# RNG65536/CUDA-volpath

Measured on AMD Instinct MI355X. Metric: Msamples/sec (WxHxspp) + achieved HBM GB/s, Julia 256^3 @ 800x600, higher is better.
Workload: dtype f32; 1 GPU; julia256_800x600_global_majorant; image=800x600, estimator=global_majorant, bound_brick=1, rng=philox2x32-7, parallelism=pixel-tiles x1

## Files before the change

### cuda-volpath_amd/csrc/vp_context.cpp

```cpp
#include "vp_state.h"

namespace vph __attribute__((visibility("hidden")))
{
State                      g_default;
static thread_local State* t_current = nullptr;
State& cur() { return t_current ? *t_current : g_default; }

int fail(int code, const char* fmt, ...)
{
    char    buf[512];
    va_list ap;
    va_start(ap, fmt);
    vsnprintf(buf, sizeof buf, fmt, ap);
    va_end(ap);
    G.err = buf;
    return code;
}
[[noreturn]] void die(const char* what)
{
    fprintf(stderr, "volpath_hip: %s: %s\n", what, G.err.c_str());
    exit(EXIT_FAILURE);
}
int ensure_device()
{
// ... 54 lines not shown
    if (knob("VP_CELL_BRICKS", 0, 1, v)) G.cell_bricks = (int)v;
    if (knob("VP_NO_CRAWL_TABLE", 0, 1, v)) G.use_crawl_table = v == 0;
    if (knob("VP_NO_EMPTY_TABLE", 0, 1, v)) G.use_empty_table = v == 0;
    if (knob("VP_NO_SUN_CLIP", 0, 1, v)) G.use_sun_clip = v == 0;
    if (knob("VP_DENSE_PERCENT", 0, 101, v)) G.dense_fraction = (float)v / 100.0f;
    if (knob("VP_NO_OPACITY_LDS", 0, 1, v)) G.opacity_lds = v == 0;
    if (knob("VP_NO_OPACITY_CELLS", 0, 1, v)) G.use_opacity_cells = v == 0;
    if (knob("VP_NO_LIGHT_CONST", 0, 1, v)) G.use_light_const = v == 0;
    if (knob("VP_NO_CONST_ROWS", 0, 1, v)) G.use_const_rows = v == 0;
    if (knob("VP_NO_APPROACH", 0, 1, v)) G.use_approach = v == 0;
    if (knob("VP_NO_APPROACH_LOCAL", 0, 1, v)) G.use_approach_local = v == 0;
    if (knob("VP_NO_APPROACH_TABLE", 0, 1, v)) G.use_approach_table = v == 0;
    if (knob("VP_NO_RAY_TABLE", 0, 1, v)) G.use_ray_table = v == 0;
    if (knob("VP_APPROACH_FRAMES_LOG2", 0, 6, v)) G.approach_fshift_max = (unsigned)v;
    if (knob("VP_APPROACH_STEPS", 0, 1 << 30, v)) G.approach_steps = (unsigned)v;
    if (knob("VP_NO_LIGHT", 0, 1, v)) G.use_light = v == 0;
    if (knob("VP_NO_LIGHT_OVERLAP", 0, 1, v)) G.light_overlap = v == 0;
    if (knob("VP_NO_LIGHT_LOCAL", 0, 1, v)) G.use_light_local = v == 0;
    if (knob("VP_DEBUG_ONLY_CLASS", 0, 1, v)) G.debug_only_class = (int)v;
    if (knob("VP_GENERAL_BLOCKS_PER_CU", 1, 8, v)) G.general_blocks_per_cu = (unsigned)v;
    if (knob("VP_LIGHT_BLOCKS_PER_CU", 1, 8, v)) G.light_blocks_per_cu = (unsigned)v;
    if (knob("VP_THR_TABLE", 2, 1 << 20, v)) G.thr_entries = (unsigned)v;
    if (knob("VP_LOOKAHEAD", 0, 4096, v)) G.la_max = (int)v;
    if (knob("VP_LOOKAHEAD_OVERLAP_FROM", 1, 4096, v)) G.la_overlap_from = (int)v;
    if (knob("VP_LOOKAHEAD_RAMP_FROM", 2, 4096, v)) G.la_ramp_from = (int)v;
    if (knob("VP_LOOKAHEAD_FLOOR", 1, 4096, v)) G.la_floor = (int)v;
    if (knob("VP_LOOKAHEAD_DIV", 1, 16, v)) G.la_div = (int)v;
    if (knob("VP_LOOKAHEAD_NO_SPECULATION", 0, 1, v)) G.la_speculate = v == 0;
    if (knob("VP_NO_LA_CANCEL", 0, 1, v)) G.la_cancel = v == 0;
    if (knob("VP_NO_PIPELINE", 0, 1, v)) G.pipeline = v == 0;
// ... 727 lines not shown
    if (!dm || !df) return fail(VP_E_NOMEM, "vp_test_log_forms: no device memory");
    HIPCHK(hipMemsetAsync(dm, 0, 8, G.stream));
    HIPCHK(hipMemsetAsync(df, 0xff, 4, G.stream));
    if (G.arith == VP_ARITH_FAST) launch_test_log_forms_fast(which, lo_bits, hi_bits, dm, df, G.stream);
    else launch_test_log_forms(which, lo_bits, hi_bits, dm, df, G.stream);
    HIPCHK(hipStreamSynchronize(G.stream));
    unsigned long long m = 0;
    HIPCHK(hipMemcpy(&m, dm, 8, hipMemcpyDeviceToHost));
    HIPCHK(hipMemcpy(first_bad, df, 4, hipMemcpyDeviceToHost));
    *mismatches = m;
    return VP_OK;
}
int vp_test_approach_walk(int kind, int n, const float* params, const uint32_t* script, const uint32_t* words, uint32_t n_words, uint32_t* out_new,
                          uint32_t* out_ref)
{
    if (kind < 0 || kind > 1) return fail(VP_E_ARG, "vp_test_approach_walk: unknown walk %d (0 approach_k's, 1 the local walks' inner loop)", kind);
    if (n < 0) return fail(VP_E_ARG, "vp_test_approach_walk: negative count %d", n);
    if (!params || !script || !out_new || !out_ref || (n_words && !words)) return fail(VP_E_ARG, "vp_test_approach_walk: null argument");
    for (int i = 0; i < n; i++)
        if (script[4 * (size_t)i + 1] > n_words || script[4 * (size_t)i + 2] > n_words - script[4 * (size_t)i + 1])
            return fail(VP_E_ARG, "vp_test_approach_walk: the script of case %d (%u words from %u) leaves the %u words given", i, script[4 * (size_t)i + 2],
                        script[4 * (size_t)i + 1], n_words);
    int rc = ensure_device();
    if (rc) return rc;
    if (n == 0) return VP_OK;
    DevArrays D;
    const size_t c = (size_t)n;
    float*    dp = (float*)D.get(c * 16);
    unsigned *ds = (unsigned*)D.get(c * 16), *dw = (unsigned*)D.get((size_t)n_words * 4), *dn = (unsigned*)D.get(c * 20), *dr = (unsigned*)D.get(c * 20);
    if (!dp || !ds || !dw || !dn || !dr) return fail(VP_E_NOMEM, "vp_test_approach_walk: no device memory");
    HIPCHK(hipMemcpy(dp, params, c * 16, hipMemcpyHostToDevice));
    HIPCHK(hipMemcpy(ds, script, c * 16, hipMemcpyHostToDevice));
    if (n_words) HIPCHK(hipMemcpy(dw, words, (size_t)n_words * 4, hipMemcpyHostToDevice));
    if (G.arith == VP_ARITH_FAST) launch_test_approach_walk_fast(kind, n, dp, ds, dw, dn, dr, G.stream);
    else launch_test_approach_walk(kind, n, dp, ds, dw, dn, dr, G.stream);
    HIPCHK(hipStreamSynchronize(G.stream));
    HIPCHK(hipMemcpy(out_new, dn, c * 20, hipMemcpyDeviceToHost));
    HIPCHK(hipMemcpy(out_ref, dr, c * 20, hipMemcpyDeviceToHost));
    return VP_OK;
}
int vp_test_sun_start(int n, const float* origin_xyz, const float* sun_dir, const float* box, uint32_t* out_new, uint32_t* out_ref)
{
    if (n < 0) return fail(VP_E_ARG, "vp_test_sun_start: negative count %d", n);
    if (!origin_xyz || !sun_dir || !box || !out_new || !out_ref) return fail(VP_E_ARG, "vp_test_sun_start: null argument");
    int rc = ensure_device();
    if (rc) return rc;
    if (n == 0) return VP_OK;
    DevArrays D;
    const size_t c = (size_t)n;
    float*    dor = (float*)D.get(c * 12), *db = (float*)D.get(24);
// ... 169 lines not shown
```

### cuda-volpath_amd/csrc/vp_integrator.h

```cpp
enum : int
{
    ST_DONE    = 0,
    ST_SETUP   = 1,
    ST_TRACK   = 2,
    ST_SHADOW  = 3,
    EV_SCATTER = 4,
    EV_NEE     = 5,
    EV_BG      = 6,
    EV_WRITE   = 7,
    EV_MIS     = 8,
    EV_HG      = 9
};

#ifndef VP_PAD_STEP
#define VP_PAD_STEP 0
#endif
#ifndef VP_PAD_FETCH
#define VP_PAD_FETCH 0
#endif
#ifndef VP_PAD_EOF
#define VP_PAD_EOF 0
#endif
#ifndef VP_PAD_SETUP
#define VP_PAD_SETUP 0
// ... 1224 lines not shown

__device__ __forceinline__ bool approach_cancelled(const LaunchDev& L)
{
    if (!L.cancel) return false;
    unsigned w = 0;
    if ((threadIdx.x & 63u) == 0u) w = __hip_atomic_load(L.cancel, __ATOMIC_RELAXED, __HIP_MEMORY_SCOPE_AGENT);
    return (unsigned)__builtin_amdgcn_readfirstlane((int)w) >= L.batch_id;
}
#define VP_KEEP_BRANCH() asm volatile("")
#define VP_WALK_UNROLL 2
__device__ __forceinline__ float walk_limit(float t_box, float t_empty) { return t_box < t_empty ? t_box : t_empty; }
__device__ __forceinline__ bool walks_backwards(float inv_sigma) { return (f2u(inv_sigma) >> 31) != 0u; }

template <class RNG>
__device__ __forceinline__ unsigned approach_walk(float& dist, const float t_lim, const float inv_sigma, const unsigned cap, RNG& rng, unsigned& sa,
                                                  unsigned& sb)
{
    unsigned steps = 0;
    rng.save(sa, sb);
    if (!RNG::kShadowSubstream || walks_backwards(inv_sigma))
    {
        for (; steps < cap; steps++)
        {
            const float d2 = dist + -logf_(rng.next_a()) * inv_sigma;
            if (!(d2 < t_lim)) break;
            dist = d2;
            (void)rng.next_b();
            rng.save(sa, sb);
        }
        return steps;
    }
    const unsigned base = sa;
    float          a = dist, b = dist;
    unsigned       twos = 0;
    bool           odd  = false;
    for (unsigned i = 0; i < cap; i += 2u)
    {
        rng.set_pair(base + i);
        const float ua = rng.next_a();
        b              = a + -logf_pos_(ua) * inv_sigma;
        if (ua == 0.0f || !(b < t_lim)) break;
        VP_KEEP_BRANCH();
        odd = true;
        if (i + 1u == cap) break;
        rng.set_pair(base + i + 1u);
        const float ub = rng.next_a();
        a              = b + -logf_pos_(ub) * inv_sigma;
        if (ub == 0.0f || !(a < t_lim)) break;
        VP_KEEP_BRANCH();
        odd = false;
        twos++;
    }
// ... 56 lines not shown
    before.set_pair(base + steps);
    before.save(ta, tb);
    return stopped && d2 >= t_far;
}

template <class RNG>
__global__ __launch_bounds__(256) void approach_k(SceneDev S, LaunchDev L)
{
    if (approach_cancelled(L)) return;
    const unsigned sh   = L.approach_fshift;
    const unsigned slot = blockIdx.x * (256u >> sh) + (threadIdx.x >> sh), fl = (blockIdx.y << sh) + (threadIdx.x & ((1u << sh) - 1u));
    if (slot >= L.nslots || fl >= (unsigned)L.nframes) return;
    const ParamDev& P = L.P;
    const unsigned pix = L.pixels[slot], px = pix & 0xffffu, py = pix >> 16;
    if (px >= P.width || py >= P.height) return;
    f3 ro, rd;
    camera_ray(S, P.width, P.height, px, py, ro, rd);
    float    t_near, tf, dist = 0.0f;
    unsigned pairs = 0, sa = 0, sb = 0;
    RNG      rng;
    if (intersect_box(ro, rd, S, t_near, tf))
    {
        if (t_near < 0.0f) t_near = 0.0f;
        dist                      = t_near;
        const float t_end         = tf;
        const float t_empty       = L.crawl[2 * ((size_t)px + (size_t)py * P.width) + 1].x;
        const float s             = hyperion_s(0 - 5);
        const float cur_density   = (1.0f - s) * P.density + s * P.density * (1.0f - P.g);
        const float sigma_t_prime = max3(f3{P.sigma_t[0], P.sigma_t[1], P.sigma_t[2]}) * cur_density;
        const float inv_sigma     = rcp_(sigma_t_prime);
        rng.init(px, py, (unsigned)(L.frame0 + (int)fl), L.key0, L.key1);
        pairs = approach_walk(dist, walk_limit(t_end, t_empty), inv_sigma, L.approach_steps, rng, sa, sb);
    }
    L.stage[(size_t)fl * L.stage_stride + L.slot_base + slot] = make_float4(dist, u2f(sa), u2f(sb), u2f(pairs));
    if (L.counters && pairs) atomicAdd(&L.counters[1], (unsigned long long)pairs);
}

template <class RNG, bool QUANT>
__global__ __launch_bounds__(256) void approach_local_k(SceneDev S, LaunchDev L)
{
    if (approach_cancelled(L)) return;
    const unsigned sh   = L.approach_fshift;
    const unsigned slot = blockIdx.x * (256u >> sh) + (threadIdx.x >> sh), fl = (blockIdx.y << sh) + (threadIdx.x & ((1u << sh) - 1u));
    if (slot >= L.nslots || fl >= (unsigned)L.nframes) return;
    const ParamDev& P = L.P;
    const unsigned pix = L.pixels[slot], px = pix & 0xffffu, py = pix >> 16;
    if (px >= P.width || py >= P.height) return;
// ... 123 lines not shown
```

### cuda-volpath_amd/csrc/vp_kernels.h

```cpp
#pragma once
#include <hip/hip_runtime.h>

#include "vp_device.h"

#define VP_BLOCK 256
#ifndef VP_BLOCK_LDS
#define VP_BLOCK_LDS 512
#endif
#ifndef VP_MIN_WAVES
#define VP_MIN_WAVES 1
#endif
#define VP_LDS_BYTES_PER_CU (160 * 1024)
#define VP_LDS_BOUND_ENTRIES 32768
#ifndef VP_CHUNK
#define VP_CHUNK 128
#endif
#define VP_NQUEUES 8
#define VP_QUEUE_STRIDE 16
#ifndef VP_WAIT_LANES
#define VP_WAIT_LANES 28
#endif
#ifndef VP_WAIT_ITERS
#define VP_WAIT_ITERS 16
#endif
// ... 61 lines not shown
    const unsigned char* exit_oct;
    int      exit_start;
    unsigned exit_nbytes;
    unsigned exit_bytes;
    unsigned* cancel;
    unsigned  batch_id;
    unsigned      const_from;
    const float4* stage_const;
    const unsigned* bound_codes;
    unsigned        bound_pal[2];
    const float4* seg_table;
    unsigned sub_shift;
    unsigned layers;
    const float4* ray;
    float4* groups;
};

[[noreturn]] void kernel_not_built();
constexpr int CENSUS_RENDER = 0, CENSUS_LAYERS = 1, CENSUS_APPROACH = 2;
void census_record(int unit, int kind, unsigned index);
size_t census_size(int kind);
void census_read(int unit, int kind, unsigned* launches, unsigned char* built, size_t count, bool reset);
void census_built(int kind, unsigned char* built, size_t count);
void census_built_fast(int kind, unsigned char* built, size_t count);
void groups_census_record(unsigned index);
void groups_census_read(unsigned* launches, unsigned char* built, size_t count, bool reset);
void group_layers_census_record(unsigned index);
void group_layers_census_read(unsigned* launches, unsigned char* built, size_t count, bool reset);
void launch_render(const SceneDev& S, const LaunchDev& L, int est, int rng, bool quant, bool half, bool count, int lds_form, bool mis, int trk,
                   int blocks, hipStream_t st);
// ... 69 lines not shown
void launch_relight_composite(float4* dst, const float4* sun, const float4* sky, const float4* trans, float3 sun_gain, float3 sky_gain, const float4* plate,
                              float r, float g, float b, int size, float s, hipStream_t st);
void launch_gamma(float4* dst, const float4* src, int size, float s, float inv_gamma, hipStream_t st);
void launch_accumulate(float4* dst, const float4* src, size_t n, hipStream_t st);
void launch_test_hg(const float* g, const float* r0, const float* r1, const float* nrm, const float* cosq, float* dir, float* ev, int n, hipStream_t st);
void launch_test_box(const SceneDev& S, const float* o, const float* d, int* hit, float* tn, float* tf, int n, hipStream_t st);
void launch_test_env(const SceneDev& S, const float* d, float* out, int n, hipStream_t st);
void launch_test_camera_ray(const SceneDev& S, unsigned width, unsigned height, const unsigned* pixels, float* dir, int n, hipStream_t st);
void launch_test_camera_ray_fast(const SceneDev& S, unsigned width, unsigned height, const unsigned* pixels, float* dir, int n, hipStream_t st);
void launch_test_math(int which, const float* in, float* out, int n, hipStream_t st);
void launch_test_roots(int which, unsigned lo, unsigned hi, unsigned long long* mismatches, unsigned* first_bad, hipStream_t st);
void launch_test_hg_fast(const float* g, const float* r0, const float* r1, const float* nrm, const float* cosq, float* dir, float* ev, int n, hipStream_t st);
void launch_test_math_fast(int which, const float* in, float* out, int n, hipStream_t st);
void launch_test_log_forms(int which, unsigned lo, unsigned hi, unsigned long long* mismatches, unsigned* first_bad, hipStream_t st);
void launch_test_log_forms_fast(int which, unsigned lo, unsigned hi, unsigned long long* mismatches, unsigned* first_bad, hipStream_t st);
void launch_test_approach_walk(int kind, int n, const float* par, const unsigned* scr, const unsigned* words, unsigned* out_new, unsigned* out_ref, hipStream_t st);
void launch_test_approach_walk_fast(int kind, int n, const float* par, const unsigned* scr, const unsigned* words, unsigned* out_new, unsigned* out_ref,
                                    hipStream_t st);
void launch_test_sun_start(int n, const float* origin, const float* sun_dir, const float* box, unsigned* out_new, unsigned* out_ref, hipStream_t st);
void launch_test_sun_start_fast(int n, const float* origin, const float* sun_dir, const float* box, unsigned* out_new, unsigned* out_ref, hipStream_t st);
void launch_test_rng(int mode, unsigned x, unsigned y, unsigned f, unsigned k0, unsigned k1, int n, float* out, hipStream_t st);
void launch_test_density(const SceneDev& S, bool quant, bool half, const float* pos, float* out, int n, hipStream_t st);
}
```

### cuda-volpath_amd/csrc/vp_kernels.hip

```cpp
#include <hip/hip_runtime.h>

#include <atomic>
#include <cmath>
#include <cstdint>
#include <cstdio>
#include <cstdlib>
#include <type_traits>
#include <utility>

#include "vp_device.h"
#include "vp_kernels.h"

namespace vp
{
#include "vp_integrator.h"

__global__ void thr_table_k(ParamDev P, float* table, unsigned count)
{
    if (threadIdx.x || blockIdx.x) return;
    const float max_sig       = max3(f3{P.sigma_t[0], P.sigma_t[1], P.sigma_t[2]});
    const float s             = hyperion_s(0 - 5);
    const float cur_density   = (1.0f - s) * P.density + s * P.density * (1.0f - P.g);
    const float sigma_t_prime = max_sig * cur_density;
    const float inv_sigma_t   = 1.0f / sigma_t_prime;
// ... 1671 lines not shown
{
    hipLaunchKernelGGL(test_env_k, dim3((n + 255) / 256), dim3(256), 0, st, S, d, out, n);
}
void launch_test_math(int which, const float* in, float* out, int n, hipStream_t st)
{
    hipLaunchKernelGGL(test_math_k, dim3((n + 255) / 256), dim3(256), 0, st, which, in, out, n);
}
void launch_test_roots(int which, unsigned lo, unsigned hi, unsigned long long* mismatches, unsigned* first_bad, hipStream_t st)
{
    hipLaunchKernelGGL(test_roots_k, dim3(2048), dim3(256), 0, st, which, lo, hi, mismatches, first_bad);
}
void launch_test_log_forms(int which, unsigned lo, unsigned hi, unsigned long long* mismatches, unsigned* first_bad, hipStream_t st)
{
    hipLaunchKernelGGL(test_log_forms_k, dim3(2048), dim3(256), 0, st, which, lo, hi, mismatches, first_bad);
}
void launch_test_approach_walk(int kind, int n, const float* par, const unsigned* scr, const unsigned* words, unsigned* out_new, unsigned* out_ref, hipStream_t st)
{
    hipLaunchKernelGGL(test_approach_walk_k, dim3((n + 63) / 64), dim3(64), 0, st, kind, n, par, scr, words, out_new, out_ref);
}
void launch_test_sun_start(int n, const float* origin, const float* sun_dir, const float* box, unsigned* out_new, unsigned* out_ref, hipStream_t st)
{
    hipLaunchKernelGGL(test_sun_start_k, dim3((n + 255) / 256), dim3(256), 0, st, n, origin, sun_dir[0], sun_dir[1], sun_dir[2], box, out_new, out_ref);
}
void launch_test_camera_ray(const SceneDev& S, unsigned width, unsigned height, const unsigned* pixels, float* dir, int n, hipStream_t st)
{
    hipLaunchKernelGGL(test_camera_ray_k, dim3((n + 255) / 256), dim3(256), 0, st, S, width, height, pixels, dir, n);
}
void launch_test_rng(int mode, unsigned x, unsigned y, unsigned f, unsigned k0, unsigned k1, int n, float* out, hipStream_t st)
{
    if (mode == RNG_PHILOX) hipLaunchKernelGGL(test_rng_k<RngPhilox>, dim3(1), dim3(64), 0, st, x, y, f, k0, k1, n, out);
    else if (mode == RNG_PHILOX7) hipLaunchKernelGGL(test_rng_k<RngPhilox7>, dim3(1), dim3(64), 0, st, x, y, f, k0, k1, n, out);
    else hipLaunchKernelGGL(test_rng_k<RngSamplerH>, dim3(1), dim3(64), 0, st, x, y, f, k0, k1, n, out);
}
// ... 8 lines not shown
```

### cuda-volpath_amd/csrc/vp_kernels_fast.hip

```cpp
#define VP_ARITH_FAST 1

#include <hip/hip_runtime.h>

#include <cstdio>
#include <cstdlib>
#include <utility>

#include "vp_device.h"
#include "vp_kernels.h"

namespace vp
{
namespace fast
{
#include "vp_integrator.h"
#include "vp_test_kernels.h"

#include "vp_dispatch.h"
}

void launch_render_fast(const SceneDev& S, const LaunchDev& L, int est, int rng, bool quant, bool half, bool count, int lds_form, bool mis, int trk,
                        int blocks, hipStream_t st)
{
    fast::dispatch_render(S, L, est, rng, quant, half, count, lds_form, mis, trk, blocks, st);
// ... 8 lines not shown
void census_built_fast(int kind, unsigned char* built, size_t count) { fast::dispatch_census_built(kind, built, count); }

void launch_test_hg_fast(const float* g, const float* r0, const float* r1, const float* nrm, const float* cosq, float* dir, float* ev, int n, hipStream_t st)
{
    hipLaunchKernelGGL(fast::test_hg_k, dim3((n + 255) / 256), dim3(256), 0, st, g, r0, r1, nrm, cosq, dir, ev, n);
}
void launch_test_math_fast(int which, const float* in, float* out, int n, hipStream_t st)
{
    hipLaunchKernelGGL(fast::test_math_k, dim3((n + 255) / 256), dim3(256), 0, st, which, in, out, n);
}
void launch_test_log_forms_fast(int which, unsigned lo, unsigned hi, unsigned long long* mismatches, unsigned* first_bad, hipStream_t st)
{
    hipLaunchKernelGGL(fast::test_log_forms_k, dim3(2048), dim3(256), 0, st, which, lo, hi, mismatches, first_bad);
}
void launch_test_approach_walk_fast(int kind, int n, const float* par, const unsigned* scr, const unsigned* words, unsigned* out_new, unsigned* out_ref,
                                    hipStream_t st)
{
    hipLaunchKernelGGL(fast::test_approach_walk_k, dim3((n + 63) / 64), dim3(64), 0, st, kind, n, par, scr, words, out_new, out_ref);
}
void launch_test_camera_ray_fast(const SceneDev& S, unsigned width, unsigned height, const unsigned* pixels, float* dir, int n, hipStream_t st)
{
    hipLaunchKernelGGL(fast::test_camera_ray_k, dim3((n + 255) / 256), dim3(256), 0, st, S, width, height, pixels, dir, n);
}
void launch_test_sun_start_fast(int n, const float* origin, const float* sun_dir, const float* box, unsigned* out_new, unsigned* out_ref, hipStream_t st)
{
    hipLaunchKernelGGL(fast::test_sun_start_k, dim3((n + 255) / 256), dim3(256), 0, st, n, origin, sun_dir[0], sun_dir[1], sun_dir[2], box, out_new, out_ref);
}
}
```

### cuda-volpath_amd/csrc/vp_render.cpp

```cpp
#include "vp_state.h"

namespace vph __attribute__((visibility("hidden")))
{
static float span_ms(hipEvent_t a, hipEvent_t b, hipEvent_t& end)
{
    float ms = 0.0f, since = 0.0f;
    if (hipEventElapsedTime(&ms, a, b) != hipSuccess) { (void)hipGetLastError(); return 0.0f; }
    if (end && hipEventElapsedTime(&since, end, b) == hipSuccess)
    {
        if (since <= 0.0f) return 0.0f;
        ms = std::min(ms, since);
    }
    else (void)hipGetLastError();
    end = b;
    return std::max(ms, 0.0f);
}
static void fold_span(hipEvent_t a, hipEvent_t b, hipEvent_t& end, double& sum)
{
    hipEvent_t e = end;
    if (hipEventQuery(b) == hipSuccess) sum += span_ms(a, b, e);
    else (void)hipGetLastError();
    put_event(a);
    if (e == b) { put_event(end); end = b; }
    else put_event(b);
// ... 312 lines not shown
}
static hipError_t launch_general_class(Launch& X, const ClassGrid& g)
{
    const LaunchPlan& A = X.A; LaunchDev& L = X.L; const Target& T = A.T;
    hipError_t le = hipSuccess;
    ClassTimer ct(0, T.stream);
    L.approach = 0;
    G.last_approach = 0;
    G.last_approach_table = 0;
    const bool aux_ok = !A.appr_aux_needed || T.rt->handover.p != nullptr;
    if (A.appr_aux_needed) L.approach_aux = T.rt->handover;
    if (A.approach && aux_ok && L.stage && X.f <= 65535)
    {
        L.approach       = A.approach_thr ? 2u : 1u;
        L.approach_steps = G.approach_steps;
        L.approach_fshift = 0;
        while (L.approach_fshift < G.approach_fshift_max && (2u << L.approach_fshift) <= (unsigned)X.f) L.approach_fshift++;
        X.k.approach(X.S, L, G.est, G.rng, G.quant, T.stream);
        le = hipGetLastError();
        G.last_approach = (int)L.approach;
        G.last_approach_table = (G.est == VP_EST_DECOMP && G.quant && L.seg_table && L.approach_fshift == 6u) ? 1 : 0;
        if (X.lds_helper && X.aux.forked && le == hipSuccess) X.aux.fork();
    }
    if (A.piped && le == hipSuccess)
    {
        if (hipEventRecord(G.pipe_gate[A.slot], T.stream) == hipSuccess) G.pipe_gate_set[A.slot] = true;
        else le = hipGetLastError();
    }
    if (le == hipSuccess)
    {
// ... 493 lines not shown
```

### cuda-volpath_amd/csrc/vp_state.h

```cpp
#pragma once
#include <hip/hip_runtime.h>

#include <cmath>
#include <cstdarg>
#include <cstdio>
#include <cstdlib>
#include <cstring>
#include <deque>
#include <string>
#include <chrono>
#include <vector>

#include "../../include/volpath.h"
#include "vp_kernels.h"

namespace vph __attribute__((visibility("hidden")))
{
using namespace vp;

inline int bound_radius(int nx, float search_radius)
{
    float cell_size = 2.0f / (float)nx;
    return (int)std::ceil(search_radius / cell_size);
}
// ... 166 lines not shown
    DevBuf<unsigned char> d_sub_cls;
    unsigned    la_launched = 0, la_cancelled = 0;
    bool        use_const_rows = true;
    unsigned    last_const_from = 0;
    bool        use_approach_table = true;
    DevBuf<float4> d_seg;
    std::vector<unsigned char> seg_key;
    bool        use_ray_table = true;
    DevBuf<float4> d_ray;
    std::vector<unsigned char> ray_key;
    int         last_ray_table = 0;
    bool        use_approach_local = true;
    bool        use_approach = true;
    unsigned    approach_fshift_max = 6;
    unsigned    approach_steps = 1u << 20;
    unsigned*   d_light_flag = nullptr;
    bool        bound_mask_valid = false;
    unsigned    h_bound_mask[8] = {};
    bool        use_exit    = true;
    bool        exit_local  = false;
    bool        exit_local_auto = true;
    unsigned    exit_k      = 8;
    unsigned char* d_exit   = nullptr;
    float       light_key[7] = {};
    unsigned long long light_epoch = ~0ull;
    bool        light_const = false;
    float       fast_identity_key[5] = {};
    bool        fast_identity_valid = false, fast_identity = false;
    float*      d_thr       = nullptr;
    float       thr_key[5]  = {};
// ... 77 lines not shown
```

### cuda-volpath_amd/csrc/vp_test_kernels.h

```cpp

__global__ void test_hg_k(const float* g, const float* r0, const float* r1, const float* nrm, const float* cosq, float* dir, float* ev, int n)
{
    int i = threadIdx.x + blockIdx.x * blockDim.x;
    if (i >= n) return;
    Frame fr(f3{nrm[3 * i], nrm[3 * i + 1], nrm[3 * i + 2]});
    f3    d = normalize(fr.to_world(hg_sample_local(g[i], r0[i], r1[i])));
    dir[3 * i] = d.x; dir[3 * i + 1] = d.y; dir[3 * i + 2] = d.z;
    ev[i] = hg_eval(g[i], cosq[i]);
}
__global__ void test_math_k(int which, const float* in, float* out, int n)
{
    int i = threadIdx.x + blockIdx.x * blockDim.x;
    if (i >= n) return;
    float x = in[i], s, c, r;
    switch (which)
    {
        case 0: r = logf_(x); break;
        case 1: r = expf_(x); break;
        case 2: sincosf_(x, s, c); r = s; break;
        case 3: sincosf_(x, s, c); r = c; break;
        case 4: r = acosf_(x); break;
        case 5: r = atanf_(x); break;
        case 6: r = pow15f_(x); break;
        case 7: r = rcp_(x); break;
// ... 85 lines not shown
                                                           unsigned& tb, unsigned& steps)
{
    bool through = false;
    for (;;)
    {
        const float d2 = dist + -logf_ref_(rng.next_a()) * inv_sigma;
        if (d2 >= t_far) { through = true; break; }
        if (!(d2 < t_empty) || steps > 60000u) break;
        dist = d2;
        (void)rng.next_b();
        rng.save(ta, tb);
        steps++;
    }
    return through;
}
__global__ void test_approach_walk_k(int kind, int n, const float* par, const unsigned* scr, const unsigned* words, unsigned* out_new, unsigned* out_ref)
{
    const int i = threadIdx.x + blockIdx.x * blockDim.x;
    if (i >= n) return;
    const float    dist0 = par[4 * i], t_empty = par[4 * i + 1], t_box = par[4 * i + 2], inv_sigma = par[4 * i + 3];
    const unsigned cap = scr[4 * i];
    for (int ref = 0; ref < 2; ref++)
    {
        RngScript rng{words + scr[4 * i + 1], scr[4 * i + 2], scr[4 * i + 3], scr[4 * i + 3]};
        float     dist = dist0;
        unsigned  sa = 0, sb = 0, steps = 0, through = 0;
        if (kind == 0)
        {
            if (ref) approach_walk_ref_(dist, t_empty, t_box, inv_sigma, cap, rng, steps, sa, sb);
            else steps = approach_walk(dist, walk_limit(t_box, t_empty), inv_sigma, cap, rng, sa, sb);
        }
        else
        {
            rng.save(sa, sb);
            if (ref) through = approach_segment_walk_ref_(dist, t_box, t_empty, inv_sigma, rng, sa, sb, steps) ? 1u : 0u;
            else
            {
                unsigned long long n_steps = 0;
                through = approach_segment_walk(dist, t_box, t_empty, inv_sigma, rng, sa, sb, n_steps) ? 1u : 0u;
                steps   = (unsigned)n_steps;
            }
        }
        unsigned* o = (ref ? out_ref : out_new) + 5 * (size_t)i;
        o[0] = f2u(dist); o[1] = steps; o[2] = sa; o[3] = sb; o[4] = through;
    }
// ... 59 lines not shown
```

### cuda-volpath_amd/volpath/__init__.py

```python
import ctypes as C
import os

import numpy as np

_HERE = os.path.dirname(os.path.abspath(__file__))
LIB_PATH = os.environ.get("VOLPATH_LIB", os.path.join(os.path.dirname(_HERE), "libvolpath_hip.so"))

EST_GLOBAL, EST_DECOMP, EST_BOUNDED = 0, 1, 2
RNG_SAMPLERH, RNG_PHILOX, RNG_PHILOX7 = 0, 1, 2
ENV_PASSIVE, ENV_MIS = 0, 1
TRACK_SPECTRAL, TRACK_SCALAR, TRACK_MULTI_CHANNEL = 0, 1, 2
ARITH_EXACT, ARITH_FAST = 0, 1
VOL_U8, VOL_F32, VOL_F16 = 0, 1, 2
ARITH_FAST_REL_L2 = 2e-3
SUBPIXEL_MAX = 8

PART1_SYMBOLS = ["init_cuda", "set_texture_filter_mode", "free_cuda_buffers", "precompute_opacity", "init_envmap",
                 "free_envmap", "set_sun", "copy_inv_view_matrix", "copy_inv_model_matrix", "init_rng", "free_rng",
                 "render_kernel", "scale", "gamma_correct"]
PART2_SYMBOLS = ["vp_last_error", "vp_version", "vp_device_count", "vp_set_device", "vp_set_stream", "vp_get_stream", "vp_synchronize",
                 "vp_set_estimator", "vp_set_rng", "vp_set_envmap_sampling", "vp_get_env_tables", "vp_set_lookahead", "vp_set_tracking", "vp_set_bound_brick", "vp_set_shard", "vp_render_frames", "vp_init_volume", "vp_get_volume_info",
                 "vp_enable_counters", "vp_read_counters", "vp_render_time_ms", "vp_get_bound_table", "vp_get_opacity", "vp_get_pixel_table", "vp_get_null_collision_table", "vp_get_sun_clip_table", "vp_get_exit_table", "vp_set_exit_flights", "vp_render_class_time_ms", "vp_last_approach_mode", "vp_last_approach_table", "vp_last_light_const", "vp_last_lds_form", "vp_set_arithmetic", "vp_last_arithmetic", "vp_set_subpixel", "vp_get_subpixel", "vp_subpixel_offset", "vp_set_pipeline", "vp_last_pipelined", "vp_lookahead_stats", "vp_prepare", "vp_reserve_frames", "vp_get_pixel_lists", "vp_get_segment_table", "vp_get_ray_table", "vp_last_ray_table",
                 "vp_render_frames_stats", "vp_render_adaptive", "vp_scale_by_count", "vp_stats_rel_error",
                 "vp_denoise", "vp_set_denoise_form", "vp_last_denoise_form",
                 "vp_render_frames_layers", "vp_composite",
                 "vp_render_frames_groups", "vp_relight", "vp_reserve_frames_groups", "vp_groups_frames_per_launch", "vp_test_groups_census",
                 "vp_render_frames_groups_stats", "vp_render_frames_layers_stats",
                 "vp_render_adaptive_groups", "vp_render_adaptive_layers",
                 "vp_render_frames_group_layers", "vp_render_frames_group_layers_stats", "vp_relight_composite", "vp_test_group_layers_census",
                 "vp_julia_voxelize", "vp_cloud_voxelize", "vp_test_math", "vp_test_rng", "vp_test_sample_density", "vp_test_hg", "vp_test_roots", "vp_test_log_forms", "vp_test_approach_walk", "vp_test_sun_start", "vp_test_launch_census", "vp_test_intersect_box", "vp_test_camera_ray",
                 "vp_test_eval_envmap", "vp_ctx_create", "vp_ctx_destroy", "vp_ctx_set_current", "vp_ctx_get_current", "vp_ctx_device",
                 "vp_accumulate", "vp_tile_owner", "vp_malloc", "vp_free", "vp_memset",
                 "vp_upload", "vp_download"]


class Float3(C.Structure):
    _fields_ = [("x", C.c_float), ("y", C.c_float), ("z", C.c_float)]


class Dim3(C.Structure):
    _fields_ = [("x", C.c_uint32), ("y", C.c_uint32), ("z", C.c_uint32)]


class VolumeInfo(C.Structure):
    _fields_ = [("format", C.c_int), ("nx", C.c_int), ("ny", C.c_int), ("nz", C.c_int), ("cell_bytes", C.c_int),
# ... 103 lines not shown
        L.vp_get_sun_clip_table.argtypes = [C.c_void_p, C.c_size_t, C.POINTER(C.c_float)]
        L.vp_render_class_time_ms.argtypes = [C.POINTER(C.c_double), C.POINTER(C.c_uint32), C.c_int]
        L.vp_prepare.argtypes = [C.POINTER(Param)]
        L.vp_set_subpixel.argtypes = [C.c_int]
        L.vp_subpixel_offset.argtypes = [C.c_uint, C.c_uint, C.c_int, C.c_int, C.POINTER(C.c_int), C.POINTER(C.c_int)]
        L.vp_get_pixel_lists.argtypes = [C.POINTER(Param), C.c_void_p, C.c_size_t, C.POINTER(C.c_uint32)]
        L.vp_get_segment_table.argtypes = [C.POINTER(Param), C.c_void_p, C.c_size_t, C.POINTER(C.c_int)]
        L.vp_get_ray_table.argtypes = [C.POINTER(Param), C.c_void_p, C.c_size_t]
        L.vp_test_camera_ray.argtypes = [C.c_uint, C.c_uint, C.c_void_p, C.c_void_p, C.c_int]
        L.vp_julia_voxelize.argtypes = [C.c_int, C.c_void_p]
        L.vp_cloud_voxelize.argtypes = [C.c_int, C.c_uint32, C.c_void_p]
        L.vp_test_math.argtypes = [C.c_int, C.c_void_p, C.c_void_p, C.c_int]
        L.vp_test_roots.argtypes = [C.c_int, C.c_uint32, C.c_uint32, C.POINTER(C.c_uint64), C.POINTER(C.c_uint32)]
        L.vp_test_log_forms.argtypes = [C.c_int, C.c_uint32, C.c_uint32, C.POINTER(C.c_uint64), C.POINTER(C.c_uint32)]
        L.vp_test_approach_walk.argtypes = [C.c_int, C.c_int, C.c_void_p, C.c_void_p, C.c_void_p, C.c_uint32, C.c_void_p, C.c_void_p]
        L.vp_test_sun_start.argtypes = [C.c_int, C.c_void_p, C.c_void_p, C.c_void_p, C.c_void_p, C.c_void_p]
        L.vp_test_launch_census.argtypes = [C.c_int, C.c_int, C.c_void_p, C.c_void_p, C.c_size_t, C.c_int]
        L.vp_test_rng.argtypes = [C.c_int] + [C.c_uint32] * 5 + [C.c_int, C.c_void_p]
        L.vp_test_sample_density.argtypes = [C.c_void_p, C.c_void_p, C.c_int]
        L.vp_test_hg.argtypes = [C.c_void_p] * 7 + [C.c_int]
        L.vp_test_intersect_box.argtypes = [C.c_void_p] * 5 + [C.c_int]
        L.vp_test_eval_envmap.argtypes = [C.c_void_p, C.c_void_p, C.c_int]
        L.vp_ctx_create.restype = C.c_void_p
        L.vp_ctx_create.argtypes = [C.c_int]
        L.vp_ctx_destroy.argtypes = [C.c_void_p]
        L.vp_ctx_set_current.argtypes = [C.c_void_p]
        L.vp_ctx_get_current.restype = C.c_void_p
        L.vp_accumulate.argtypes = [C.c_void_p, C.c_void_p, C.c_size_t]
        L.vp_tile_owner.argtypes = [C.c_uint, C.c_uint, C.c_int]
        L.init_cuda.argtypes = [C.c_void_p, Extent, C.c_bool, C.POINTER(Float3), C.POINTER(Float3)]
# ... 492 lines not shown
    return out


def test_roots(which, lo_bits, hi_bits):
    m, f = C.c_uint64(0), C.c_uint32(0)
    _chk(lib().vp_test_roots(which, lo_bits, hi_bits, C.byref(m), C.byref(f)))
    return m.value, (None if m.value == 0 else f.value)


def test_log_forms(which, lo_bits, hi_bits):
    m, f = C.c_uint64(0), C.c_uint32(0)
    _chk(lib().vp_test_log_forms(which, lo_bits, hi_bits, C.byref(m), C.byref(f)))
    return m.value, (None if m.value == 0 else f.value)


def test_approach_walk(kind, params, script, words):
    params = np.ascontiguousarray(params, np.float32).reshape(-1, 4)
    script = np.ascontiguousarray(script, np.uint32).reshape(-1, 4)
    words = np.ascontiguousarray(words, np.uint32).ravel()
    n = params.shape[0]
    if script.shape[0] != n:
        raise ValueError("params and script describe different numbers of cases")
    new, ref = np.zeros((n, 5), np.uint32), np.zeros((n, 5), np.uint32)
    _chk(lib().vp_test_approach_walk(kind, n, _p(params), _p(script), _p(words), words.size, _p(new), _p(ref)))
    return new, ref


def test_sun_start(origins, sun_dir, box):
    origins = np.ascontiguousarray(origins, np.float32).reshape(-1, 3)
    sun_dir = np.ascontiguousarray(sun_dir, np.float32).ravel()
    box = np.ascontiguousarray(box, np.float32).ravel()
    if sun_dir.size != 3 or box.size != 6:
        raise ValueError("sun_dir has three components, box six (bmin, bmax)")
    n = origins.shape[0]
    new, ref = np.zeros((n, 8), np.uint32), np.zeros((n, 8), np.uint32)
    _chk(lib().vp_test_sun_start(n, _p(origins), _p(sun_dir), _p(box), _p(new), _p(ref)))
    return new, ref


# ... 142 lines not shown
```

### include/volpath.h

```cpp
#ifndef VOLPATH_H
#define VOLPATH_H

#include <stddef.h>
#include <stdint.h>
#ifndef __cplusplus
#include <stdbool.h>
#endif

#ifdef __cplusplus
extern "C" {
#endif

typedef struct { float x, y, z; } vp_float3;
typedef struct { float x, y, z, w; } vp_float4;
typedef struct { uint32_t x, y, z; } vp_dim3;
typedef struct { size_t width, height, depth; } vp_extent;

#ifndef VOLPATH_PARAM_DEFINED
#define VOLPATH_PARAM_DEFINED
typedef struct Param
{
    unsigned int width, height;
    float        density, brightness;
    vp_float3    albedo;
// ... 162 lines not shown
int vp_get_pixel_table(const Param* p, float* dst, size_t count);
int vp_get_segment_table(const Param* p, float* dst, size_t count, int* cap);
int vp_get_ray_table(const Param* p, float* dst, size_t count);
int vp_last_ray_table(void);
int vp_test_camera_ray(unsigned width, unsigned height, const uint32_t* pixels, float* out, int n);
int vp_get_sun_clip_table(unsigned short* dst, size_t count, float* step);
int vp_get_exit_table(unsigned char* dst, size_t count);
int vp_set_exit_flights(int mode);
int vp_get_null_collision_table(const Param* p, float* dst, size_t count);

int vp_test_math(int which, const float* in, float* out, int n);
int vp_test_roots(int which, uint32_t lo_bits, uint32_t hi_bits, uint64_t* mismatches, uint32_t* first_bad);
int vp_test_log_forms(int which, uint32_t lo_bits, uint32_t hi_bits, uint64_t* mismatches, uint32_t* first_bad);
int vp_test_approach_walk(int kind, int n, const float* params, const uint32_t* script, const uint32_t* words, uint32_t n_words,
                          uint32_t* out_new, uint32_t* out_ref);
int vp_test_sun_start(int n, const float* origin_xyz, const float* sun_dir, const float* box, uint32_t* out_new, uint32_t* out_ref);
int vp_test_launch_census(int unit, int kind, uint32_t* launches, uint8_t* built, size_t count, int reset);
int vp_test_groups_census(uint32_t* launches, uint8_t* built, size_t count, int reset);
int vp_test_group_layers_census(uint32_t* launches, uint8_t* built, size_t count, int reset);
int vp_test_rng(int mode, uint32_t x, uint32_t y, uint32_t frame, uint32_t k0, uint32_t k1, int n, float* out);
int vp_test_sample_density(const float* pos_xyz, float* out, int n);
int vp_test_hg(const float* g, const float* r0, const float* r1, const float* normal_xyz, const float* cos_query, float* dir_xyz,
               float* eval, int n);
int vp_test_intersect_box(const float* origin_xyz, const float* dir_xyz, int* hit, float* tnear, float* tfar, int n);
int vp_test_eval_envmap(const float* dir_xyz, float* rgb, int n);

int vp_julia_voxelize(int n, unsigned char* host_out);
int vp_cloud_voxelize(int n, uint32_t seed, float* host_out);

void* vp_malloc(size_t bytes);
// ... 10 lines not shown
```

Before: 3726 Msamples/s.

## Cut approach walk short when few wavefront lanes remain; read precomputed ray table

The approach pre-walk loop now checks the active-lane count each iteration with a wavefront ballot and stops when fewer than a tail threshold (default 12) lanes are still walking. The remaining walk then falls to the main tracking kernel, which resumes from the saved RNG state and distance. The approach kernel also reads t_near, t_far and t_empty from the precomputed ray table when one is available, skipping camera-ray generation, box intersection and the crawl lookup. This targets divergent tail iterations where most lanes of a wave are idle, at the cost of a ballot per iteration and more leftover work for the next stage.

```diff
diff --git a/cuda-volpath_amd/csrc/vp_context.cpp b/cuda-volpath_amd/csrc/vp_context.cpp
--- a/cuda-volpath_amd/csrc/vp_context.cpp
+++ b/cuda-volpath_amd/csrc/vp_context.cpp
@@ -92,6 +92,7 @@
     if (knob("VP_NO_RAY_TABLE", 0, 1, v)) G.use_ray_table = v == 0;
     if (knob("VP_APPROACH_FRAMES_LOG2", 0, 6, v)) G.approach_fshift_max = (unsigned)v;
     if (knob("VP_APPROACH_STEPS", 0, 1 << 30, v)) G.approach_steps = (unsigned)v;
+    if (knob("VP_APPROACH_TAIL", 0, 64, v)) G.approach_tail = (unsigned)v;
     if (knob("VP_NO_LIGHT", 0, 1, v)) G.use_light = v == 0;
     if (knob("VP_NO_LIGHT_OVERLAP", 0, 1, v)) G.light_overlap = v == 0;
     if (knob("VP_NO_LIGHT_LOCAL", 0, 1, v)) G.use_light_local = v == 0;
@@ -849,6 +850,12 @@
 int vp_test_approach_walk(int kind, int n, const float* params, const uint32_t* script, const uint32_t* words, uint32_t n_words, uint32_t* out_new,
                           uint32_t* out_ref)
 {
+    return vp_test_approach_walk_tail(kind, n, params, script, words, n_words, 0u, out_new, out_ref);
+}
+int vp_test_approach_walk_tail(int kind, int n, const float* params, const uint32_t* script, const uint32_t* words, uint32_t n_words, uint32_t tail,
+                               uint32_t* out_new, uint32_t* out_ref)
+{
+    if (tail > 64u) return fail(VP_E_ARG, "vp_test_approach_walk: tail %u (allowed 0..64)", tail);
     if (kind < 0 || kind > 1) return fail(VP_E_ARG, "vp_test_approach_walk: unknown walk %d (0 approach_k's, 1 the local walks' inner loop)", kind);
     if (n < 0) return fail(VP_E_ARG, "vp_test_approach_walk: negative count %d", n);
     if (!params || !script || !out_new || !out_ref || (n_words && !words)) return fail(VP_E_ARG, "vp_test_approach_walk: null argument");
@@ -867,8 +874,8 @@
     HIPCHK(hipMemcpy(dp, params, c * 16, hipMemcpyHostToDevice));
     HIPCHK(hipMemcpy(ds, script, c * 16, hipMemcpyHostToDevice));
     if (n_words) HIPCHK(hipMemcpy(dw, words, (size_t)n_words * 4, hipMemcpyHostToDevice));
-    if (G.arith == VP_ARITH_FAST) launch_test_approach_walk_fast(kind, n, dp, ds, dw, dn, dr, G.stream);
-    else launch_test_approach_walk(kind, n, dp, ds, dw, dn, dr, G.stream);
+    if (G.arith == VP_ARITH_FAST) launch_test_approach_walk_fast(kind, n, dp, ds, dw, dn, dr, G.stream, tail);
+    else launch_test_approach_walk(kind, n, dp, ds, dw, dn, dr, G.stream, tail);
     HIPCHK(hipStreamSynchronize(G.stream));
     HIPCHK(hipMemcpy(out_new, dn, c * 20, hipMemcpyDeviceToHost));
     HIPCHK(hipMemcpy(out_ref, dr, c * 20, hipMemcpyDeviceToHost));
diff --git a/cuda-volpath_amd/csrc/vp_integrator.h b/cuda-volpath_amd/csrc/vp_integrator.h
--- a/cuda-volpath_amd/csrc/vp_integrator.h
+++ b/cuda-volpath_amd/csrc/vp_integrator.h
@@ -1262,7 +1262,7 @@
 
 template <class RNG>
 __device__ __forceinline__ unsigned approach_walk(float& dist, const float t_lim, const float inv_sigma, const unsigned cap, RNG& rng, unsigned& sa,
-                                                  unsigned& sb)
+                                                  unsigned& sb, const unsigned tail = 0u)
 {
     unsigned steps = 0;
     rng.save(sa, sb);
@@ -1284,6 +1284,7 @@
     bool           odd  = false;
     for (unsigned i = 0; i < cap; i += 2u)
     {
+        if ((unsigned)__builtin_popcountll(__builtin_amdgcn_ballot_w64(true)) < tail) break;
         rng.set_pair(base + i);
         const float ua = rng.next_a();
         b              = a + -logf_pos_(ua) * inv_sigma;
@@ -1370,23 +1371,36 @@
     const ParamDev& P = L.P;
     const unsigned pix = L.pixels[slot], px = pix & 0xffffu, py = pix >> 16;
     if (px >= P.width || py >= P.height) return;
-    f3 ro, rd;
-    camera_ray(S, P.width, P.height, px, py, ro, rd);
-    float    t_near, tf, dist = 0.0f;
+    float    t_near, tf, t_empty, dist = 0.0f;
+    bool     hit;
+    if (L.ray && !L.sub_shift)
+    {
+        const float4 e0 = L.ray[2 * (size_t)slot], e1 = L.ray[2 * (size_t)slot + 1];
+        t_near  = e0.w;
+        tf      = e1.x;
+        t_empty = e1.y;
+        hit     = tf > t_near && tf >= 1e-3f;
+    }
+    else
+    {
+        f3 ro, rd;
+        camera_ray(S, P.width, P.height, px, py, ro, rd);
+        hit     = intersect_box(ro, rd, S, t_near, tf);
+        t_empty = hit ? L.crawl[2 * ((size_t)px + (size_t)py * P.width) + 1].x : 0.0f;
+    }
     unsigned pairs = 0, sa = 0, sb = 0;
     RNG      rng;
-    if (intersect_box(ro, rd, S, t_near, tf))
+    if (hit)
     {
         if (t_near < 0.0f) t_near = 0.0f;
         dist                      = t_near;
         const float t_end         = tf;
-        const float t_empty       = L.crawl[2 * ((size_t)px + (size_t)py * P.width) + 1].x;
         const float s             = hyperion_s(0 - 5);
         const float cur_density   = (1.0f - s) * P.density + s * P.density * (1.0f - P.g);
         const float sigma_t_prime = max3(f3{P.sigma_t[0], P.sigma_t[1], P.sigma_t[2]}) * cur_density;
         const float inv_sigma     = rcp_(sigma_t_prime);
         rng.init(px, py, (unsigned)(L.frame0 + (int)fl), L.key0, L.key1);
-        pairs = approach_walk(dist, walk_limit(t_end, t_empty), inv_sigma, L.approach_steps, rng, sa, sb);
+        pairs = approach_walk(dist, walk_limit(t_end, t_empty), inv_sigma, L.approach_steps, rng, sa, sb, L.approach_tail);
     }
     L.stage[(size_t)fl * L.stage_stride + L.slot_base + slot] = make_float4(dist, u2f(sa), u2f(sb), u2f(pairs));
     if (L.counters && pairs) atomicAdd(&L.counters[1], (unsigned long long)pairs);
diff --git a/cuda-volpath_amd/csrc/vp_kernels.h b/cuda-volpath_amd/csrc/vp_kernels.h
--- a/cuda-volpath_amd/csrc/vp_kernels.h
+++ b/cuda-volpath_amd/csrc/vp_kernels.h
@@ -99,6 +99,7 @@
     unsigned layers;
     const float4* ray;
     float4* groups;
+    unsigned approach_tail;
 };
 
 [[noreturn]] void kernel_not_built();
@@ -198,9 +199,10 @@
 void launch_test_math_fast(int which, const float* in, float* out, int n, hipStream_t st);
 void launch_test_log_forms(int which, unsigned lo, unsigned hi, unsigned long long* mismatches, unsigned* first_bad, hipStream_t st);
 void launch_test_log_forms_fast(int which, unsigned lo, unsigned hi, unsigned long long* mismatches, unsigned* first_bad, hipStream_t st);
-void launch_test_approach_walk(int kind, int n, const float* par, const unsigned* scr, const unsigned* words, unsigned* out_new, unsigned* out_ref, hipStream_t st);
+void launch_test_approach_walk(int kind, int n, const float* par, const unsigned* scr, const unsigned* words, unsigned* out_new, unsigned* out_ref, hipStream_t st,
+                               unsigned tail = 0u);
 void launch_test_approach_walk_fast(int kind, int n, const float* par, const unsigned* scr, const unsigned* words, unsigned* out_new, unsigned* out_ref,
-                                    hipStream_t st);
+                                    hipStream_t st, unsigned tail = 0u);
 void launch_test_sun_start(int n, const float* origin, const float* sun_dir, const float* box, unsigned* out_new, unsigned* out_ref, hipStream_t st);
 void launch_test_sun_start_fast(int n, const float* origin, const float* sun_dir, const float* box, unsigned* out_new, unsigned* out_ref, hipStream_t st);
 void launch_test_rng(int mode, unsigned x, unsigned y, unsigned f, unsigned k0, unsigned k1, int n, float* out, hipStream_t st);
diff --git a/cuda-volpath_amd/csrc/vp_kernels.hip b/cuda-volpath_amd/csrc/vp_kernels.hip
--- a/cuda-volpath_amd/csrc/vp_kernels.hip
+++ b/cuda-volpath_amd/csrc/vp_kernels.hip
@@ -1709,9 +1709,9 @@
 {
     hipLaunchKernelGGL(test_log_forms_k, dim3(2048), dim3(256), 0, st, which, lo, hi, mismatches, first_bad);
 }
-void launch_test_approach_walk(int kind, int n, const float* par, const unsigned* scr, const unsigned* words, unsigned* out_new, unsigned* out_ref, hipStream_t st)
-{
-    hipLaunchKernelGGL(test_approach_walk_k, dim3((n + 63) / 64), dim3(64), 0, st, kind, n, par, scr, words, out_new, out_ref);
+void launch_test_approach_walk(int kind, int n, const float* par, const unsigned* scr, const unsigned* words, unsigned* out_new, unsigned* out_ref, hipStream_t st, unsigned tail)
+{
+    hipLaunchKernelGGL(test_approach_walk_k, dim3((n + 63) / 64), dim3(64), 0, st, kind, n, par, scr, words, out_new, out_ref, tail);
 }
 void launch_test_sun_start(int n, const float* origin, const float* sun_dir, const float* box, unsigned* out_new, unsigned* out_ref, hipStream_t st)
 {
diff --git a/cuda-volpath_amd/csrc/vp_kernels_fast.hip b/cuda-volpath_amd/csrc/vp_kernels_fast.hip
--- a/cuda-volpath_amd/csrc/vp_kernels_fast.hip
+++ b/cuda-volpath_amd/csrc/vp_kernels_fast.hip
@@ -46,9 +46,9 @@
     hipLaunchKernelGGL(fast::test_log_forms_k, dim3(2048), dim3(256), 0, st, which, lo, hi, mismatches, first_bad);
 }
 void launch_test_approach_walk_fast(int kind, int n, const float* par, const unsigned* scr, const unsigned* words, unsigned* out_new, unsigned* out_ref,
-                                    hipStream_t st)
+                                    hipStream_t st, unsigned tail)
 {
-    hipLaunchKernelGGL(fast::test_approach_walk_k, dim3((n + 63) / 64), dim3(64), 0, st, kind, n, par, scr, words, out_new, out_ref);
+    hipLaunchKernelGGL(fast::test_approach_walk_k, dim3((n + 63) / 64), dim3(64), 0, st, kind, n, par, scr, words, out_new, out_ref, tail);
 }
 void launch_test_camera_ray_fast(const SceneDev& S, unsigned width, unsigned height, const unsigned* pixels, float* dir, int n, hipStream_t st)
 {
diff --git a/cuda-volpath_amd/csrc/vp_render.cpp b/cuda-volpath_amd/csrc/vp_render.cpp
--- a/cuda-volpath_amd/csrc/vp_render.cpp
+++ b/cuda-volpath_amd/csrc/vp_render.cpp
@@ -350,6 +350,7 @@
     {
         L.approach       = A.approach_thr ? 2u : 1u;
         L.approach_steps = G.approach_steps;
+        L.approach_tail  = G.approach_tail;
         L.approach_fshift = 0;
         while (L.approach_fshift < G.approach_fshift_max && (2u << L.approach_fshift) <= (unsigned)X.f) L.approach_fshift++;
         X.k.approach(X.S, L, G.est, G.rng, G.quant, T.stream);
diff --git a/cuda-volpath_amd/csrc/vp_state.h b/cuda-volpath_amd/csrc/vp_state.h
--- a/cuda-volpath_amd/csrc/vp_state.h
+++ b/cuda-volpath_amd/csrc/vp_state.h
@@ -204,6 +204,7 @@
     bool        use_approach = true;
     unsigned    approach_fshift_max = 6;
     unsigned    approach_steps = 1u << 20;
+    unsigned    approach_tail = 12;
     unsigned*   d_light_flag = nullptr;
     bool        bound_mask_valid = false;
     unsigned    h_bound_mask[8] = {};
diff --git a/cuda-volpath_amd/csrc/vp_test_kernels.h b/cuda-volpath_amd/csrc/vp_test_kernels.h
--- a/cuda-volpath_amd/csrc/vp_test_kernels.h
+++ b/cuda-volpath_amd/csrc/vp_test_kernels.h
@@ -123,7 +123,8 @@
     }
     return through;
 }
-__global__ void test_approach_walk_k(int kind, int n, const float* par, const unsigned* scr, const unsigned* words, unsigned* out_new, unsigned* out_ref)
+__global__ void test_approach_walk_k(int kind, int n, const float* par, const unsigned* scr, const unsigned* words, unsigned* out_new, unsigned* out_ref,
+                                     unsigned tail)
 {
     const int i = threadIdx.x + blockIdx.x * blockDim.x;
     if (i >= n) return;
@@ -137,7 +138,7 @@
         if (kind == 0)
         {
             if (ref) approach_walk_ref_(dist, t_empty, t_box, inv_sigma, cap, rng, steps, sa, sb);
-            else steps = approach_walk(dist, walk_limit(t_box, t_empty), inv_sigma, cap, rng, sa, sb);
+            else steps = approach_walk(dist, walk_limit(t_box, t_empty), inv_sigma, cap, rng, sa, sb, tail);
         }
         else
         {
diff --git a/cuda-volpath_amd/volpath/__init__.py b/cuda-volpath_amd/volpath/__init__.py
--- a/cuda-volpath_amd/volpath/__init__.py
+++ b/cuda-volpath_amd/volpath/__init__.py
@@ -28,7 +28,7 @@
                  "vp_render_frames_groups_stats", "vp_render_frames_layers_stats",
                  "vp_render_adaptive_groups", "vp_render_adaptive_layers",
                  "vp_render_frames_group_layers", "vp_render_frames_group_layers_stats", "vp_relight_composite", "vp_test_group_layers_census",
-                 "vp_julia_voxelize", "vp_cloud_voxelize", "vp_test_math", "vp_test_rng", "vp_test_sample_density", "vp_test_hg", "vp_test_roots", "vp_test_log_forms", "vp_test_approach_walk", "vp_test_sun_start", "vp_test_launch_census", "vp_test_intersect_box", "vp_test_camera_ray",
+                 "vp_julia_voxelize", "vp_cloud_voxelize", "vp_test_math", "vp_test_rng", "vp_test_sample_density", "vp_test_hg", "vp_test_roots", "vp_test_log_forms", "vp_test_approach_walk", "vp_test_approach_walk_tail", "vp_test_sun_start", "vp_test_launch_census", "vp_test_intersect_box", "vp_test_camera_ray",
                  "vp_test_eval_envmap", "vp_ctx_create", "vp_ctx_destroy", "vp_ctx_set_current", "vp_ctx_get_current", "vp_ctx_device",
                  "vp_accumulate", "vp_tile_owner", "vp_malloc", "vp_free", "vp_memset",
                  "vp_upload", "vp_download"]
@@ -162,6 +162,7 @@
         L.vp_test_roots.argtypes = [C.c_int, C.c_uint32, C.c_uint32, C.POINTER(C.c_uint64), C.POINTER(C.c_uint32)]
         L.vp_test_log_forms.argtypes = [C.c_int, C.c_uint32, C.c_uint32, C.POINTER(C.c_uint64), C.POINTER(C.c_uint32)]
         L.vp_test_approach_walk.argtypes = [C.c_int, C.c_int, C.c_void_p, C.c_void_p, C.c_void_p, C.c_uint32, C.c_void_p, C.c_void_p]
+        L.vp_test_approach_walk_tail.argtypes = [C.c_int, C.c_int, C.c_void_p, C.c_void_p, C.c_void_p, C.c_uint32, C.c_uint32, C.c_void_p, C.c_void_p]
         L.vp_test_sun_start.argtypes = [C.c_int, C.c_void_p, C.c_void_p, C.c_void_p, C.c_void_p, C.c_void_p]
         L.vp_test_launch_census.argtypes = [C.c_int, C.c_int, C.c_void_p, C.c_void_p, C.c_size_t, C.c_int]
         L.vp_test_rng.argtypes = [C.c_int] + [C.c_uint32] * 5 + [C.c_int, C.c_void_p]
@@ -684,7 +685,7 @@
     return m.value, (None if m.value == 0 else f.value)
 
 
-def test_approach_walk(kind, params, script, words):
+def test_approach_walk(kind, params, script, words, tail=0):
     params = np.ascontiguousarray(params, np.float32).reshape(-1, 4)
     script = np.ascontiguousarray(script, np.uint32).reshape(-1, 4)
     words = np.ascontiguousarray(words, np.uint32).ravel()
@@ -692,7 +693,7 @@
     if script.shape[0] != n:
         raise ValueError("params and script describe different numbers of cases")
     new, ref = np.zeros((n, 5), np.uint32), np.zeros((n, 5), np.uint32)
-    _chk(lib().vp_test_approach_walk(kind, n, _p(params), _p(script), _p(words), words.size, _p(new), _p(ref)))
+    _chk(lib().vp_test_approach_walk_tail(kind, n, _p(params), _p(script), _p(words), words.size, tail, _p(new), _p(ref)))
     return new, ref
 
 
diff --git a/include/volpath.h b/include/volpath.h
--- a/include/volpath.h
+++ b/include/volpath.h
@@ -200,6 +200,8 @@
 int vp_test_log_forms(int which, uint32_t lo_bits, uint32_t hi_bits, uint64_t* mismatches, uint32_t* first_bad);
 int vp_test_approach_walk(int kind, int n, const float* params, const uint32_t* script, const uint32_t* words, uint32_t n_words,
                           uint32_t* out_new, uint32_t* out_ref);
+int vp_test_approach_walk_tail(int kind, int n, const float* params, const uint32_t* script, const uint32_t* words, uint32_t n_words,
+                               uint32_t tail, uint32_t* out_new, uint32_t* out_ref);
 int vp_test_sun_start(int n, const float* origin_xyz, const float* sun_dir, const float* box, uint32_t* out_new, uint32_t* out_ref);
 int vp_test_launch_census(int unit, int kind, uint32_t* launches, uint8_t* built, size_t count, int reset);
 int vp_test_groups_census(uint32_t* launches, uint8_t* built, size_t count, int reset);
```

Result: no change. 3726 Msamples/s, median of 2 (-0.0%).
